# Vanlightly/vsr-tlaplus

Hardware: AMD Instinct MI355X
Metric: distinct states/sec (whole node) + time-to-first-violation, VSR 3-replica (higher is better)
Workload: dtype u64

## Files before the change

include/vsrmc.h:

```cpp
#ifndef VSRMC_H
#define VSRMC_H
#include <stdint.h>

#ifdef __cplusplus
extern "C" {
#endif

#define VSRMC_E_ARG (-1)
#define VSRMC_E_CFG (-2)
#define VSRMC_E_HIP (-3)
#define VSRMC_E_EVAL (-4)
#define VSRMC_E_REP (-5)
#define VSRMC_E_STATE (-6)

typedef struct vsrmc_model vsrmc_model;
typedef struct vsrmc_fpset vsrmc_fpset;
typedef struct vsrmc_checker vsrmc_checker;

const char* vsrmc_last_error(void);
int32_t vsrmc_version(void);
int32_t vsrmc_device_count(void);

typedef struct vsrmc_layout {
  int32_t replica_count, client_count, value_count, start_view_on_timer_limit;
// ... 217 lines not shown
  uint64_t min_fp[8], min_index[8];
  uint32_t min_ordinal[8];
  int32_t min_action[8];
  double kernel_ms, list_ms, apply_ms;
  uint64_t slices;
} vsrmc_step_info;
int32_t vsrmc_step_compile(const vsrmc_model* m, const char* text, vsrmc_where** out);
int32_t vsrmc_step_predicates_compile(const vsrmc_model* m, const char* text, vsrmc_where** out);
int32_t vsrmc_step_batch(const vsrmc_model* m, int32_t device, const vsrmc_where* w, const uint64_t* words, const uint64_t* off, uint64_t n, uint64_t* rows,
                         uint64_t cap_rows, uint64_t* n_rows);
int32_t vsrmc_checker_step_scan(vsrmc_checker* c, const vsrmc_where* w, vsrmc_step_info* out);
int32_t vsrmc_checker_step_successor(vsrmc_checker* c, uint64_t index, uint32_t ordinal, const uint64_t* parent, uint64_t parent_words, uint64_t* words,
                                     uint64_t cap_words, uint64_t* n_words, int32_t* action);
int32_t vsrmc_checker_step_pairs(vsrmc_checker* c, uint64_t* fps, uint32_t* ordinals, uint8_t* bits, uint64_t cap, uint64_t* n);

int32_t vsrmc_checker_probe(vsrmc_checker* c, vsrmc_level_info* info);
int32_t vsrmc_checker_probe2(vsrmc_checker* c, vsrmc_level_info* virt, vsrmc_level_info* probe);
int32_t vsrmc_checker_probe3(vsrmc_checker* c, vsrmc_level_info* virt1, vsrmc_level_info* virt2, vsrmc_level_info* probe);
int32_t vsrmc_checker_deepen(vsrmc_checker* c, vsrmc_level_info* inserted, vsrmc_level_info* probed);
int32_t vsrmc_checker_advance(vsrmc_checker* c, vsrmc_level_info* a, vsrmc_level_info* b, int32_t* what);
int32_t vsrmc_checker_room(vsrmc_checker* c, int32_t* state);
int32_t vsrmc_checker_probe_candidates(vsrmc_checker* c, uint64_t* pairs, uint64_t cap_pairs, uint64_t* n);
int32_t vsrmc_checker_probe_violators(vsrmc_checker* c, uint64_t* fps, uint64_t cap, uint64_t* n);
int32_t vsrmc_checker_seen_batch(vsrmc_checker* c, const uint64_t* fps, uint64_t n, int32_t level, uint8_t* seen);
int32_t vsrmc_checker_probe_trace(vsrmc_checker* c, uint64_t* words, uint64_t cap_words, uint64_t* off, int32_t* actions,
                                  uint64_t cap_states, uint64_t* n_states);
int32_t vsrmc_checker_trace_to_violator(vsrmc_checker* c, uint64_t fp, uint64_t* words, uint64_t cap_words, uint64_t* off, int32_t* actions,
                                        uint64_t cap_states, uint64_t* n_states);

typedef struct vsrmc_deep_info {
  int32_t level, kind;
  int32_t exact;
  int32_t has_state, has_step, reserved0;
  uint64_t slices;
  uint64_t n_hit_states, n_hit_pairs;
  double where_ms, step_ms;
} vsrmc_deep_info;
int32_t vsrmc_checker_deep_attach(vsrmc_checker* c, const vsrmc_where* state_prog, const vsrmc_where* step_prog);
int32_t vsrmc_checker_deep_levels(vsrmc_checker* c, int32_t* levels, int32_t* probed, uint64_t cap, uint64_t* n);
int32_t vsrmc_checker_deep_result(vsrmc_checker* c, int32_t level, int32_t probed, vsrmc_deep_info* info, vsrmc_where_info* w, vsrmc_step_info* s);
int32_t vsrmc_checker_deep_where_states(vsrmc_checker* c, int32_t level, int32_t probed, uint64_t* fps, uint8_t* bits, uint64_t cap, uint64_t* n);
int32_t vsrmc_checker_deep_step_pairs(vsrmc_checker* c, int32_t level, uint64_t* fps, uint32_t* ordinals, uint8_t* bits, uint64_t cap, uint64_t* n);
int32_t vsrmc_checker_deep_witness(vsrmc_checker* c, int32_t level, int32_t which_program, int32_t k, uint64_t* words, uint64_t cap_words, uint64_t* off,
                                   int32_t* actions, uint64_t cap_states, uint64_t* n_states);

typedef struct vsrmc_deep_terminal_info {
// ... 129 lines not shown
```

vsr_tlaplus_amd/capi.py:

```python
import ctypes as C
import os

HERE = os.path.dirname(os.path.abspath(__file__))
LIB_PATH = os.environ.get("VSRMC_LIB") or os.path.join(HERE, "libvsrmc.so")

u64p = C.POINTER(C.c_uint64)


class Layout(C.Structure):
    _fields_ = [(n, C.c_int32) for n in (
        "replica_count", "client_count", "value_count", "start_view_on_timer_limit", "symmetry", "invariant_mask",
        "assume_commit_number", "check_deadlock", "words_per_replica", "fixed_words", "permutations", "max_bag",
        "max_record_words", "module")] + [("reserved", C.c_int32 * 2)]


class Options(C.Structure):
    _fields_ = [("device", C.c_int32), ("table_log2", C.c_int32), ("frontier_words", C.c_uint64),
                ("frontier_states", C.c_uint64), ("pending_entries", C.c_uint64), ("keep_trace", C.c_int32),
                ("rank", C.c_int32), ("world", C.c_int32), ("trace_entries", C.c_uint64), ("exact_ties", C.c_int32), ("filter_log2", C.c_int32), ("host_frontier", C.c_int32), ("reserved0", C.c_int32), ("frontier_words_b", C.c_uint64)]


class LevelInfo(C.Structure):
    _fields_ = [("level", C.c_int32), ("error_code", C.c_int32), ("frontier", C.c_uint64), ("generated", C.c_uint64),
                ("n_new", C.c_uint64), ("distinct", C.c_uint64), ("total_generated", C.c_uint64),
# ... 189 lines not shown
    "vsrmc_checker_deep_terminal_states": (C.c_int32, [V, C.c_int32, C.c_int32, V, V, C.c_uint64, C.POINTER(C.c_uint64)]),
    "vsrmc_checker_deep_terminal_witness": (C.c_int32, [V, C.c_int32, C.c_int32, C.c_int32, V, C.c_uint64, V, V, C.c_uint64, C.POINTER(C.c_uint64)]),
    "vsrmc_check": (C.c_int32, [V, C.c_int32, C.c_double, C.POINTER(C.c_int32), C.POINTER(LevelInfo)]),
    "vsrmc_queue_create": (C.c_int32, [C.c_int32, C.c_uint64, C.c_uint64, C.POINTER(V)]),
    "vsrmc_queue_enqueue_batch": (C.c_int32, [V, V, V, C.c_uint64]),
    "vsrmc_queue_dequeue_batch": (C.c_int32, [V, C.c_uint64, V, C.c_uint64, V, C.POINTER(C.c_uint64)]),
    "vsrmc_queue_size": (C.c_int32, [V, C.POINTER(C.c_uint64)]),
    "vsrmc_queue_destroy": (None, [V]),
    "vsrmc_simulate": (C.c_int32, [V, C.c_int32, C.c_uint32, C.c_int32, C.c_uint64, C.c_double, C.POINTER(SimResult)]),
    "vsrmc_simulate_where": (C.c_int32, [V, C.c_int32, V, V, C.c_int32, C.c_uint32, C.c_int32, C.c_uint64, C.c_double, C.c_uint64,
                                         C.POINTER(SimWhereResult)]),
    "vsrmc_simulate_constrained": (C.c_int32, [V, C.c_int32, V, C.c_int32, V, C.c_int32, C.c_uint32, C.c_int32, C.c_uint32, C.c_int32, C.c_uint64,
                                               C.c_double, C.c_uint64, C.POINTER(SimConstrainedResult)]),
    "vsrmc_checker_probe": (C.c_int32, [V, C.POINTER(LevelInfo)]),
    "vsrmc_checker_probe2": (C.c_int32, [V, C.POINTER(LevelInfo), C.POINTER(LevelInfo)]),
    "vsrmc_checker_probe3": (C.c_int32, [V, C.POINTER(LevelInfo), C.POINTER(LevelInfo), C.POINTER(LevelInfo)]),
    "vsrmc_checker_deepen": (C.c_int32, [V, C.POINTER(LevelInfo), C.POINTER(LevelInfo)]),
    "vsrmc_checker_options": (C.c_int32, [V, C.POINTER(Options)]),
    "vsrmc_checker_advance": (C.c_int32, [V, C.POINTER(LevelInfo), C.POINTER(LevelInfo), C.POINTER(C.c_int32)]),
    "vsrmc_checker_room": (C.c_int32, [V, C.POINTER(C.c_int32)]),
    "vsrmc_checker_probe_candidates": (C.c_int32, [V, C.c_void_p, C.c_uint64, C.POINTER(C.c_uint64)]),
    "vsrmc_checker_seen_batch": (C.c_int32, [V, C.c_void_p, C.c_uint64, C.c_int32, C.c_void_p]),
    "vsrmc_checker_probe_violators": (C.c_int32, [V, C.c_void_p, C.c_uint64, C.POINTER(C.c_uint64)]),
    "vsrmc_checker_probe_trace": (C.c_int32, [V, V, C.c_uint64, V, V, C.c_uint64, C.POINTER(C.c_uint64)]),
    "vsrmc_checker_bench_staging": (C.c_int32, [V, C.c_int32, C.c_int32, C.POINTER(C.c_double), C.POINTER(C.c_uint64)]),
    "vsrmc_checker_trace_to_violator": (C.c_int32, [V, C.c_uint64, V, C.c_uint64, V, V, C.c_uint64, C.POINTER(C.c_uint64)]),
    "vsrmc_checker_save": (C.c_int32, [V, C.c_char_p]),
    "vsrmc_checker_status": (C.c_int32, [V, C.POINTER(LevelInfo)]),
    "vsrmc_checker_load": (C.c_int32, [V, C.POINTER(Options), C.c_char_p, C.POINTER(V)]),
    "vsrmc_model_parse_states": (C.c_int32, [V, C.c_char_p, V, C.c_uint64, V, V, C.c_uint64, C.POINTER(C.c_uint64)]),
    "vsrmc_model_check_trace": (C.c_int32, [V, C.c_int32, V, V, C.c_uint64, V, V, C.POINTER(C.c_int64), C.POINTER(C.c_int32)]),
    "vsrmc_shard_expand": (C.c_int32, [V, C.POINTER(ShardIO), V]),
    "vsrmc_shard_claim": (C.c_int32, [V, V, C.c_uint64, V]),
    "vsrmc_shard_materialize": (C.c_int32, [V, C.POINTER(ShardIO), V]),
    "vsrmc_shard_count": (C.c_int32, [V, C.POINTER(C.c_uint64), C.POINTER(C.c_uint64)]),
    "vsrmc_shard_export": (C.c_int32, [V, C.c_uint64, C.c_uint64, V, C.c_uint64, V, V, C.c_uint64, C.POINTER(C.c_uint64),
                                      C.POINTER(C.c_uint64)]),
    "vsrmc_shard_append": (C.c_int32, [V, V, C.c_uint64, V, V, C.c_uint64]),
    "vsrmc_shard_commit": (C.c_int32, [V, C.POINTER(LevelInfo)]),
    "vsrmc_shard_local_step": (C.c_int32, [V, C.POINTER(LevelInfo)]),
    "vsrmc_shard_partition": (C.c_int32, [V, C.POINTER(C.c_uint64)]),
    "vsrmc_shard_set_max_bag": (C.c_int32, [V, C.c_uint64]),
    "vsrmc_comm_rccl_unique_id": (C.c_int32, [V]),
    "vsrmc_comm_rccl_create": (C.c_int32, [V, C.c_int32, C.c_int32, C.c_int32, C.POINTER(C.POINTER(Comm))]),
    "vsrmc_comm_rccl_destroy": (None, [C.POINTER(Comm)]),
    "vsrmc_shard_loop_create": (C.c_int32, [V, C.POINTER(Comm), C.c_uint64, C.c_uint64, C.c_uint64, C.c_uint64, C.POINTER(V)]),
# ... 73 lines not shown
```

vsr_tlaplus_amd/checker.py:

```python
import ctypes as C
import os

import numpy as np

from . import capi
from .capi import VsrmcError, check

ACTION_NAMES = ["Initial predicate", "TimerSendSVC", "ReceiveHigherSVC", "ReceiveMatchingSVC", "SendDVC",
                "ReceiveHigherDVC", "ReceiveMatchingDVC", "SendSV", "ReceiveSV", "ReceiveClientRequest",
                "ReceivePrepareMsg", "ReceivePrepareOkMsg", "ExecuteOp", "SendGetState", "ReceiveGetState",
                "ReceiveNewState"]

INV_ACK_NOT_LOST = 1
INV_ACK_ON_MAJORITY = 2


def _p(a):
    return C.c_void_p(a.ctypes.data)


class Where:

    def __init__(self, handle, model):
        self._h = handle
# ... 1146 lines not shown
            self.violation = dict(level=d["level"], index=None, fp=d["viol_fp"], mask=d["viol_mask"], probed=True)
        return d

    def probe2(self):
        v, p = capi.LevelInfo(), capi.LevelInfo()
        check(capi.load().vsrmc_checker_probe2(self._h, C.byref(v), C.byref(p)))
        dv, dp = v.as_dict(), p.as_dict()
        for d in (dv, dp):
            d["ancestor_index"] = d.pop("viol_index")
            if d["viol_mask"] and self.violation is None:
                self.violation = dict(level=d["level"], index=None, fp=d["viol_fp"], mask=d["viol_mask"], probed=True)
        return dv, dp

    def probe3(self):
        v1, v2, p = capi.LevelInfo(), capi.LevelInfo(), capi.LevelInfo()
        check(capi.load().vsrmc_checker_probe3(self._h, C.byref(v1), C.byref(v2), C.byref(p)))
        out = [v1.as_dict(), v2.as_dict(), p.as_dict()]
        for d in out:
            d["ancestor_index"] = d.pop("viol_index")
            if d["viol_mask"] and self.violation is None:
                self.violation = dict(level=d["level"], index=None, fp=d["viol_fp"], mask=d["viol_mask"], probed=True)
        return tuple(out)

    def probe_violators(self):
        n = C.c_uint64()
        check(capi.load().vsrmc_checker_probe_violators(self._h, None, 0, C.byref(n)))
        out = np.zeros(max(1, n.value), dtype=np.uint64)
        check(capi.load().vsrmc_checker_probe_violators(self._h, _p(out), len(out), C.byref(n)))
        return [int(x) for x in out[: n.value]]

    def probe_trace(self):
        lay = self.model.layout
        n_max = max(self.level, self.depth) + 3
        cap_w = (n_max + 1) * int(lay.max_record_words)
        words = np.zeros(cap_w, dtype=np.uint64)
        off = np.zeros(n_max + 2, dtype=np.uint64)
        acts = np.zeros(n_max + 2, dtype=np.int32)
        n = C.c_uint64()
        check(capi.load().vsrmc_checker_probe_trace(self._h, _p(words), cap_w, _p(off), _p(acts), len(off), C.byref(n)))
        return [(ACTION_NAMES[acts[t]], words[int(off[t]): int(off[t + 1])].copy()) for t in range(n.value)]

    def trace_to_violator(self, fp):
        lay = self.model.layout
        n_max = max(self.level, self.depth) + 3
        cap_w = (n_max + 1) * int(lay.max_record_words)
        words = np.zeros(cap_w, dtype=np.uint64)
# ... 17 lines not shown
```

vsr_tlaplus_amd/csrc/host_checker.hpp:

```cpp
#pragma once

struct PassDst {
  u64* words = nullptr;
  u64 words_cap = 0;
  u64* off = nullptr;
  u64* fp = nullptr;
  u64 cap = 0;
  bool own_words = true;
  bool own_index = true;
};
struct DeepLevelRec { u64 n_new = 0, n_local = 0, generated = 0, max_bag = 0, frontier = 0; };
struct vsrmc_deep_attach;
struct vsrmc_deep_terminal;
struct vsrmc_constraint;
struct vsrmc_action_constraint;
struct vsrmc_checker {
  vsrmc_model model;
  vsrmc_options opt;
  hipStream_t stream = nullptr;
  hipEvent_t ev[4] = {nullptr, nullptr, nullptr, nullptr};
  Slot* table = nullptr;
  u64 tmask = 0;
  u64* words[2] = {nullptr, nullptr};
  u64* off[2] = {nullptr, nullptr};
// ... 12 lines not shown
  double t_level0 = 0, expand_ms = 0, materialize_ms = 0;
  u64 nx_n = 0, nx_w = 0;
  u64 n_valid = 1;
  u64 cur_w = 0;
  u64* rslot = nullptr;
  u64 rslot_cap = 0;
  u64* filter = nullptr;
  u64 fmask = 0;
  u64* cand_idx = nullptr;
  u64 cand_idx_cap = 0;
  bool level_fused = false;
  int failed_code = 0;
  void* fused_kernel = nullptr;
  void* plain_kernel = nullptr;
  u64* redo_buf[2] = {nullptr, nullptr};
  void* plain5_kernel = nullptr;
  void* modes_kernel = nullptr;
  void* regen_bits_kernel = nullptr, *insert_kernel = nullptr;
  void* probe_kernel = nullptr;
  void* probe_scan_kernel = nullptr, *probe_apply_kernel = nullptr;
  u64* probe_list = nullptr;
  u64 probe_list_cap = 0;
  bool probe_scan_off = false;
  u64 cur_max_bag = 0;
  bool bag_known = true;
  u64 probe_fp = 0, probe_extra_fp = 0;
  int probe_level = 0;
  std::vector<u64> probe_viol;
  std::vector<u64> probe_viol_key;
  int probe_viol_level = 0;
  int host_frontier = 0;
  bool saw_violation = false;
  u64 extra_launches = 0;
  bool probe_all_actions = false;
  int deep = 0;
  std::vector<DeepLevelRec> deep_lv;
  u64 deep_g = 2;
  u64 deep_distinct = 0, deep_generated = 0;
  bool deep_regen_done = false;
  bool rebase_off = false;
  std::vector<PassDst> scratch;
  PassDst scratch0;
  bool scratch_carved = false;
  int scratch_buf = -1;
  u64 scratch_front = 0;
  WSet h_wset = {nullptr, nullptr, 0};
// ... 50 lines not shown
double constraint_write_ratio(const vsrmc_checker* c);
bool deep_constrain_on(const vsrmc_checker* c);
int deep_constrain_filtered_through(const vsrmc_checker* c);
int deep_constrain_begin(vsrmc_checker* c, int first, int last);
int deep_constrain_slice(vsrmc_checker* c, const PassDst& B, u64 part, int level, ConstrainCtl* inserted);
int deep_constrain_end(vsrmc_checker* c, int rc, int base, int last_regen);
void deep_constrain_drop_empty(vsrmc_checker* c);
u64 deep_constrain_pruned_of(const vsrmc_checker* c, int level);
int phase_expand_gated(vsrmc_checker* c);
void action_constraint_restart(vsrmc_checker* c);
void action_constraint_free(vsrmc_checker* c);
int action_constraint_trace(vsrmc_checker* c, const std::vector<u64>& fps, u64* words, u64 cap_words, u64* off, int32_t* actions, u64 cap_states, u64* n_states);
const vsrmc_where* action_constraint_program(const vsrmc_checker* c, int* k);
bool action_deep_on(const vsrmc_checker* c);
int expand_pass_gated(vsrmc_checker* c, const u64* src_words, const u64* src_off, u64 n, u64 p_off, int level, int mode, u64 bag, const PassDst* dst);
void action_deep_file(vsrmc_checker* c, int level, int kind);
void action_deep_epoch(vsrmc_checker* c);
typedef void (*ExpandKernel)(Model, const u64*, const u64*, u64, int, int, Slot*, u64, u64*, u64, LevelCtl*, int, int, u64*, u64, u32, u64*,
                             u64, u64*, u64, u64*, u32, u32, int, u32, u64*, u64, u64*, u32, int, u64, const WSet*, u32);
typedef void (*MaterializeKernel)(Model, const u64*, const u64*, const u64*, u64, Slot*, u64*, u64, u64*, u64, u64*, LevelCtl*,
                                  const uint8_t*, u64*, u64*, int, u32, u32, int, const u64*);
typedef void (*ProbeScanKernel)(Model, const u64*, const u64*, u64, LevelCtl*, int, u32, u64*, u64);
typedef void (*ProbeApplyKernel)(Model, const u64*, const u64*, const u64*, u64, u64*, u64, LevelCtl*);
struct KernelSet {
  ExpandKernel exact;
  MaterializeKernel materialize;
  ExpandKernel fused;
  bool generic;
  ExpandKernel plain = nullptr, plain5 = nullptr, modes = nullptr, regen_bits = nullptr, insert = nullptr, probe = nullptr;
  ProbeScanKernel scan = nullptr;
  ProbeApplyKernel apply = nullptr;
};
template <int SPEC>
KernelSet full_set(ExpandKernel plain5 = nullptr) {
  KernelSet k{k_expand<false, SPEC>, k_materialize<SPEC>, k_expand<true, SPEC>, false, k_expand<true, SPEC, EXPAND_PLAIN>, plain5,
              k_expand<true, SPEC, EXPAND_MODES>, k_expand<true, SPEC, EXPAND_REGEN_BITS>, k_expand<true, SPEC, EXPAND_INSERT>};
  if constexpr ((SPEC % 1000) / 100 <= 3) { k.scan = k_probe_scan<SPEC>; k.apply = k_probe_apply<SPEC>; }
  else k.probe = k_expand<true, SPEC, EXPAND_PROBE>;
  return k;
}
KernelSet kernels_for(const Model& M) {
  switch (M.model_id * 1000 + M.R * 100 + M.C * 10 + M.n) {
    case 211: return {k_expand<false, 211>, k_materialize<211>, k_expand<true, 211>, false};
    case 212: return {k_expand<false, 0>, k_materialize<0>, k_expand<true, 212>, false};
    case 311: return {k_expand<false, 0>, k_materialize<0>, k_expand<true, 311>, false};
    case 312: return full_set<312>(k_expand<true, 312, EXPAND_PLAIN5>);
    case 313: return full_set<313>();
    case 323: {
      KernelSet k{k_expand<false, 0>, k_materialize<0>, k_expand<true, 323>, false};
      k.plain = k_expand<true, 323, EXPAND_PLAIN>;
      return k;
    }
    case 412: return {k_expand<false, 0>, k_materialize<0>, k_expand<true, 412>, false};
    case 512: return full_set<512>();
    case 1302: {
      KernelSet k{k_expand<false, 1000>, k_materialize<1000>, k_expand<true, 1302>, false};
      k.plain = k_expand<true, 1302, EXPAND_PLAIN>;
      return k;
    }
    case 2302: {
// ... 302 lines not shown
    vsrmc_checker_destroy(c);
    return fail(VSRMC_E_HIP, std::string("hipMalloc: ") + hipGetErrorString(e));
  }
  const KernelSet ks = kernels_for(M);
  c->fused_kernel = (void*)ks.fused;
  c->modes_kernel = (void*)ks.modes;
  c->plain_kernel = (void*)ks.plain;
  c->plain5_kernel = (void*)ks.plain5;
  c->regen_bits_kernel = (void*)ks.regen_bits;
  c->insert_kernel = (void*)ks.insert;
  c->probe_kernel = std::getenv("VSRMC_NO_PROBE_KERNEL") ? nullptr : (void*)ks.probe;
  if (ks.scan && ks.apply && !std::getenv("VSRMC_NO_PROBE_KERNEL")) {
    u64 cap = std::max<u64>((u64)1 << 12, std::min<u64>((u64)1 << 24, o->frontier_states / 4));
    if (const char* ev = std::getenv("VSRMC_PROBE_LIST")) cap = (u64)std::max<long long>(1, std::atoll(ev));
    if (hipMalloc((void**)&c->probe_list, ((u64)PSCAN_LIST_HDR + cap) * 8) == hipSuccess) {
      c->probe_list_cap = cap;
      c->probe_scan_kernel = (void*)ks.scan;
      c->probe_apply_kernel = (void*)ks.apply;
    } else {
      (void)hipGetLastError();
      c->probe_list = nullptr;
    }
  }
  rc = checker_seed(c);
  if (rc) { vsrmc_checker_destroy(c); return rc; }
  *out = c;
  return 0;
}

int32_t vsrmc_checker_options(const vsrmc_checker* c, vsrmc_options* out) {
  if (!c || !out) return fail(VSRMC_E_ARG, "NULL argument");
  *out = c->opt;
  return 0;
}

int32_t vsrmc_checker_reset(vsrmc_checker* c) {
  if (!c) return fail(VSRMC_E_ARG, "NULL argument");
  return checker_seed(c);
}

}

namespace {

int level_error(vsrmc_checker* c, const LevelCtl& h, int new_level) {
  c->failed = 1;
// ... 432 lines not shown
        return rrc;
      }
      return probe_pass_finish(c, src_words, src_off, level);
    }
    u32 cchunk = 0;
    if (io) {
      if (c->cand_idx_cap < (u64)c->opt.world * io->cand_cap) {
        if (c->cand_idx) (void)hipFree(c->cand_idx);
        c->cand_idx = nullptr;
        c->cand_idx_cap = 0;
        HIPCHK(hipMalloc((void**)&c->cand_idx, (u64)c->opt.world * io->cand_cap * 8));
        c->cand_idx_cap = (u64)c->opt.world * io->cand_cap;
      }
      cchunk = (u32)std::max<u64>(16, std::min<u64>(512, io->cand_cap / (4 * (u64)c->num_cus * 2)));
    }
    const int tile = fs.tile;
    const u64 ntiles = (n_parents + tile - 1) / tile;
    const u32 ccap = fs.ccap;
    const size_t lds = fs.lds;
    const int nxt = c->cur ^ 1;
    u64* const d_words = dst ? dst->words : c->words[nxt];
    u64* const d_off = dst ? dst->off : c->off[nxt];
    u64* const d_fp = dst ? dst->fp : c->lvl_fp;
    const u64 d_wcap = dst ? dst->words_cap : c->words_cap(nxt);
    const u64 nx_cap = dst ? dst->cap : c->opt.frontier_states;
    unsigned grid = (unsigned)std::min<u64>(ntiles, (u64)c->num_cus * fs.blocks_per_cu);
    grid = (unsigned)std::max<u64>(1, std::min<u64>(grid, std::min<u64>(nx_cap / (4 * (u64)VSR_CAND_CAP), d_wcap / (4 * 16384))));
    const u64 wmin = std::max<u64>(16384, (u64)ccap * (u64)(fs.stride + 5));
    grid = (unsigned)std::max<u64>(1, std::min<u64>(grid, d_wcap / (4 * wmin)));
    const u64 ichunk_max = (dst || mode == MODE_REGEN) ? std::max<u64>(VSR_CAND_CAP, 2048) : 8192;
    const u32 ichunk = (u32)std::max<u64>(VSR_CAND_CAP, std::min<u64>(ichunk_max, nx_cap / (4 * (u64)grid)));
    const u32 wchunk = (u32)std::max<u64>(std::min<u64>(wmin, d_wcap / 2), std::min<u64>(262144, d_wcap / (4 * (u64)grid)));
    HIPCHK(hipEventRecord(c->ev[0], c->stream));
    const void* kern = !one_rank ? c->fused_kernel : (use_plain || use_probe) ? fs.kernel : (c->modes_kernel ? c->modes_kernel : c->fused_kernel);
    if (!claim_bits && c->claim_bits && one_rank && level == c->level + 1 && (mode == MODE_INSERT || mode == MODE_REGEN) &&
        p_offset + n_parents <= c->claim_parents) { claim_bits = c->claim_bits; claim_w = c->claim_w; }
    if (one_rank && !use_plain) {
      if (mode == MODE_REGEN && claim_bits && c->regen_bits_kernel && claim_w <= 2 * (u64)(VSR_BLOCK / fs.tile)) kern = c->regen_bits_kernel;
      else if (mode == MODE_INSERT && c->insert_kernel) kern = c->insert_kernel;
    }
    if (claim_bits && kern != c->regen_bits_kernel && kern != c->insert_kernel) { claim_bits = nullptr; claim_w = 0; }
    if (use_plain || use_probe) { redo_kern = kern; redo_stride = fs.stride; redo_ichunk = ichunk; redo_wchunk = wchunk; redo_words = d_words; redo_off = d_off; redo_fp = d_fp; redo_wcap = d_wcap; redo_cap = nx_cap; redo_grid = grid; }
    hipLaunchKernelGGL((ExpandKernel)kern, dim3(grid), dim3(VSR_BLOCK), lds, c->stream, M, src_words, src_off, n_parents, level, c->opt.rank,
                       c->table, c->tmask, c->pending, c->opt.pending_entries, c->ctl, fs.stride, io ? c->opt.world : 1,
                       io ? io->cand_send : nullptr, io ? io->cand_cap : (u64)0, (u32)VSR_CAND_CAP,
                       d_words, d_wcap, d_off, nx_cap, d_fp,
                       ichunk, wchunk, tile, ccap, !one_rank ? c->filter : (u64*)claim_bits, !one_rank ? c->fmask : claim_w, io ? c->cand_idx : nullptr, cchunk,
                       mode | ((mode == MODE_PROBE && (c->saw_violation || c->probe_all_actions)) ? (int)MODE_NO_FOOTPRINT : 0), p_offset,
                       (const WSet*)((io && c->opt.world > 1) ? c->d_wset : nullptr), c->wepoch);
    HIPCHK(hipGetLastError());
    HIPCHK(hipEventRecord(c->ev[1], c->stream));
  }
  HIPCHK(hipMemcpyAsync(&c->h, c->ctl, sizeof(c->h), hipMemcpyDeviceToHost, c->stream));
  HIPCHK(hipStreamSynchronize(c->stream));
  if (n_parents > 0) {
    float ms = 0;
    HIPCHK(hipEventElapsedTime(&ms, c->ev[0], c->ev[1]));
    c->expand_ms += ms;
  }
  if (redo_kern && !use_probe && c->h.n_redo && !c->h.err) {
    const int rrc = redo_overflowed_tiles(c, redo_kern, src_words, src_off, level, redo_stride, redo_words, redo_wcap, redo_off, redo_cap, redo_fp, redo_ichunk, redo_wchunk, redo_grid);
    if (rrc) return rrc;
  }
  if (use_probe && c->h.n_redo > c->h.redo_cap && !c->h.err) c->h.err = ERR_FRONTIER_FULL;
  if (use_probe && c->h.n_redo && !c->h.err) {
    const int rrc = redo_overflowed_tiles(c, c->probe_kernel, src_words, src_off, level, redo_stride, redo_words, redo_wcap, redo_off, redo_cap, redo_fp, redo_ichunk, redo_wchunk,
                                          redo_grid, MODE_PROBE, probe_ccap);
    if (rrc) return rrc;
  }
  if (use_probe && c->h.err == ERR_FRONTIER_FULL) {
    void* const pk = c->probe_kernel;
    const u64 before = c->extra_launches + 1;
// ... 61 lines not shown
```

vsr_tlaplus_amd/csrc/host_search.hpp:

```cpp
#pragma once

extern "C" {

int32_t vsrmc_checker_probe(vsrmc_checker* c, vsrmc_level_info* info) {
  if (!c || !info) return fail(VSRMC_E_ARG, "NULL argument");
  if (c->opt.exact_ties) return fail(VSRMC_E_STATE, "probe levels need a single-pass checker");
  if (c->constraint && !deep_constrain_on(c)) return fail(VSRMC_E_STATE, "vsrmc_checker_probe: a constraint is attached (vsrmc_checker_constrain_attach): the levels beyond the record buffers are not constrained");
  if (c->action_constraint && !action_deep_on(c)) return fail(VSRMC_E_STATE, "vsrmc_checker_probe: an action constraint is attached (vsrmc_checker_action_constrain_attach): the levels beyond the record buffers are not constrained");
  if (c->action_constraint && c->constraint) return fail(VSRMC_E_STATE, "vsrmc_checker_probe: a state constraint beside an action constraint that is applied beyond the record buffers: the two together are not taken there");
  if (c->failed && c->failed_code != ERR_FRONTIER_FULL) return fail(VSRMC_E_STATE, "the checker stopped on an error");
  c->failed = 0;
  c->probe_fp = 0;
  c->probe_level = 0;
  c->probe_extra_fp = 0;
  c->probe_viol.clear();
  c->probe_viol_key.clear();
  c->probe_viol_level = 0;
  const bool gated = action_deep_on(c);
  int rc = 0;
  if (gated) {
    HIPCHK(hipSetDevice(c->opt.device));
    c->t_level0 = now_s();
    c->expand_ms = 0;
    action_deep_epoch(c);
// ... 60 lines not shown
  return 0;
}

int32_t vsrmc_checker_probe_candidates(vsrmc_checker* c, uint64_t* pairs, uint64_t cap_pairs, uint64_t* n) {
  if (!c || !n) return fail(VSRMC_E_ARG, "NULL argument");
  *n = c->h.n_pending;
  if (c->h.n_pending > c->opt.pending_entries) return fail(VSRMC_E_REP, "more violating successors than the pending list holds (pending_entries)");
  if (c->h.n_pending == 0 || !pairs) return 0;
  if (cap_pairs < c->h.n_pending) return fail(VSRMC_E_ARG, "buffer too small");
  HIPCHK(hipSetDevice(c->opt.device));
  HIPCHK(hipMemcpy(pairs, c->pending, 16 * c->h.n_pending, hipMemcpyDeviceToHost));
  return 0;
}

int32_t vsrmc_checker_probe_violators(vsrmc_checker* c, uint64_t* fps, uint64_t cap, uint64_t* n) {
  if (!c || !n) return fail(VSRMC_E_ARG, "NULL argument");
  *n = (u64)c->probe_viol.size();
  if (!fps) return 0;
  if (cap < *n) return fail(VSRMC_E_ARG, "buffer too small");
  for (u64 i = 0; i < *n; i++) fps[i] = c->probe_viol[(size_t)i];
  return 0;
}

int32_t vsrmc_checker_seen_batch(vsrmc_checker* c, const uint64_t* fps, uint64_t n, int32_t level, uint8_t* seen) {
  if (!c || (n && (!fps || !seen))) return fail(VSRMC_E_ARG, "NULL argument");
  if (n == 0) return 0;
  HIPCHK(hipSetDevice(c->opt.device));
  u64* d = nullptr;
  HIPCHK(hipMalloc((void**)&d, 16 * n));
  std::vector<u64> flags(n, 0);
  hipError_t e = hipMemcpy(d, fps, 8 * n, hipMemcpyHostToDevice);
  if (e == hipSuccess) {
    hipLaunchKernelGGL(k_table_seen, dim3((unsigned)((n + 255) / 256)), dim3(256), 0, c->stream, c->table, c->tmask, d, (u64)n, (int)level, d + n);
    e = hipGetLastError();
  }
  if (e == hipSuccess) e = hipStreamSynchronize(c->stream);
  if (e == hipSuccess) e = hipMemcpy(flags.data(), d + n, 8 * n, hipMemcpyDeviceToHost);
  (void)hipFree(d);
  if (e != hipSuccess) return fail(VSRMC_E_HIP, std::string("vsrmc_checker_seen_batch: ") + hipGetErrorString(e));
  for (u64 i = 0; i < n; i++) seen[i] = flags[i] ? 1 : 0;
  return 0;
}

int32_t vsrmc_checker_probe_trace(vsrmc_checker* c, uint64_t* words, uint64_t cap_words, uint64_t* off, int32_t* actions,
                                  uint64_t cap_states, uint64_t* n_states) {
  if (!c || !words || !off || !actions || !n_states) return fail(VSRMC_E_ARG, "NULL argument");
// ... 286 lines not shown
```

vsr_tlaplus_amd/csrc/vsrmc.hip:

```cpp
#include <algorithm>
#include <chrono>
#include <cstdio>
#include <cstdlib>
#include <cstring>
#include <fstream>
#include <map>
#include <sstream>
#include <string>
#include <vector>

#include "../../include/vsrmc.h"
#include "vsr_format.hpp"
#include "vrst_format.hpp"
#include "vras_format.hpp"
#include "vsr_parse.hpp"
#include "vras_parse.hpp"
#include "vsr_kernels.hpp"
#include "vsr_probe_scan.hpp"
#include "vsr_terminal.hpp"
#include "vsr_where.hpp"
#include "vsr_constrain.hpp"
#include "vsr_deep_constrain.hpp"
#include "vsr_where_parse.hpp"
#include "vsr_step.hpp"
#include "vsr_action_constrain.hpp"
#include "vsr_deep_where.hpp"
#include "vsr_deep_terminal.hpp"
#include "vsr_sim_where.hpp"
#include "vsr_sim_constrain.hpp"

#define VSRMC_FP_VERSION 2

using namespace vsr;

namespace {

thread_local std::string g_err;

int fail(int code, const std::string& msg) {
  g_err = msg;
  return code;
// ... 86 lines not shown
```

Measured before the change: 1.838 billion.

## Add dedicated wave-parallel regen-bits kernel driven by claim bitmaps

```diff
diff --git a/include/vsrmc.h b/include/vsrmc.h
--- a/include/vsrmc.h
+++ b/include/vsrmc.h
@@ -263,6 +263,7 @@
 int32_t vsrmc_checker_room(vsrmc_checker* c, int32_t* state);
 int32_t vsrmc_checker_probe_candidates(vsrmc_checker* c, uint64_t* pairs, uint64_t cap_pairs, uint64_t* n);
 int32_t vsrmc_checker_probe_violators(vsrmc_checker* c, uint64_t* fps, uint64_t cap, uint64_t* n);
+int32_t vsrmc_checker_regen_launches(const vsrmc_checker* c, uint64_t* n);
 int32_t vsrmc_checker_seen_batch(vsrmc_checker* c, const uint64_t* fps, uint64_t n, int32_t level, uint8_t* seen);
 int32_t vsrmc_checker_probe_trace(vsrmc_checker* c, uint64_t* words, uint64_t cap_words, uint64_t* off, int32_t* actions,
                                   uint64_t cap_states, uint64_t* n_states);
diff --git a/vsr_tlaplus_amd/capi.py b/vsr_tlaplus_amd/capi.py
--- a/vsr_tlaplus_amd/capi.py
+++ b/vsr_tlaplus_amd/capi.py
@@ -235,6 +235,7 @@
     "vsrmc_checker_probe_candidates": (C.c_int32, [V, C.c_void_p, C.c_uint64, C.POINTER(C.c_uint64)]),
     "vsrmc_checker_seen_batch": (C.c_int32, [V, C.c_void_p, C.c_uint64, C.c_int32, C.c_void_p]),
     "vsrmc_checker_probe_violators": (C.c_int32, [V, C.c_void_p, C.c_uint64, C.POINTER(C.c_uint64)]),
+    "vsrmc_checker_regen_launches": (C.c_int32, [V, C.POINTER(C.c_uint64)]),
     "vsrmc_checker_probe_trace": (C.c_int32, [V, V, C.c_uint64, V, V, C.c_uint64, C.POINTER(C.c_uint64)]),
     "vsrmc_checker_bench_staging": (C.c_int32, [V, C.c_int32, C.c_int32, C.POINTER(C.c_double), C.POINTER(C.c_uint64)]),
     "vsrmc_checker_trace_to_violator": (C.c_int32, [V, C.c_uint64, V, C.c_uint64, V, V, C.c_uint64, C.POINTER(C.c_uint64)]),
diff --git a/vsr_tlaplus_amd/checker.py b/vsr_tlaplus_amd/checker.py
--- a/vsr_tlaplus_amd/checker.py
+++ b/vsr_tlaplus_amd/checker.py
@@ -1192,6 +1192,11 @@
                 self.violation = dict(level=d["level"], index=None, fp=d["viol_fp"], mask=d["viol_mask"], probed=True)
         return tuple(out)
 
+    def regen_launches(self):
+        n = C.c_uint64()
+        check(capi.load().vsrmc_checker_regen_launches(self._h, C.byref(n)))
+        return n.value
+
     def probe_violators(self):
         n = C.c_uint64()
         check(capi.load().vsrmc_checker_probe_violators(self._h, None, 0, C.byref(n)))
diff --git a/vsr_tlaplus_amd/csrc/host_checker.hpp b/vsr_tlaplus_amd/csrc/host_checker.hpp
--- a/vsr_tlaplus_amd/csrc/host_checker.hpp
+++ b/vsr_tlaplus_amd/csrc/host_checker.hpp
@@ -58,6 +58,10 @@
   u64* probe_list = nullptr;
   u64 probe_list_cap = 0;
   bool probe_scan_off = false;
+  void* regen_kernel = nullptr;
+  u32 regen_trip = 64;
+  u64 regen_launches = 0;
+  u64 regen_dst_states = 0, regen_dst_words = 0;
   u64 cur_max_bag = 0;
   bool bag_known = true;
   u64 probe_fp = 0, probe_extra_fp = 0;
@@ -154,6 +158,7 @@
                                   const uint8_t*, u64*, u64*, int, u32, u32, int, const u64*);
 typedef void (*ProbeScanKernel)(Model, const u64*, const u64*, u64, LevelCtl*, int, u32, u64*, u64);
 typedef void (*ProbeApplyKernel)(Model, const u64*, const u64*, const u64*, u64, u64*, u64, LevelCtl*);
+typedef void (*RegenBitsKernel)(Model, const u64*, const u64*, u64, u64, const u32*, u32, LevelCtl*, int, u32, u32, u64*, u64, u64*, u64, u64*, u32, u32);
 struct KernelSet {
   ExpandKernel exact;
   MaterializeKernel materialize;
@@ -162,12 +167,13 @@
   ExpandKernel plain = nullptr, plain5 = nullptr, modes = nullptr, regen_bits = nullptr, insert = nullptr, probe = nullptr;
   ProbeScanKernel scan = nullptr;
   ProbeApplyKernel apply = nullptr;
+  RegenBitsKernel regen = nullptr;
 };
 template <int SPEC>
 KernelSet full_set(ExpandKernel plain5 = nullptr) {
   KernelSet k{k_expand<false, SPEC>, k_materialize<SPEC>, k_expand<true, SPEC>, false, k_expand<true, SPEC, EXPAND_PLAIN>, plain5,
               k_expand<true, SPEC, EXPAND_MODES>, k_expand<true, SPEC, EXPAND_REGEN_BITS>, k_expand<true, SPEC, EXPAND_INSERT>};
-  if constexpr ((SPEC % 1000) / 100 <= 3) { k.scan = k_probe_scan<SPEC>; k.apply = k_probe_apply<SPEC>; }
+  if constexpr ((SPEC % 1000) / 100 <= 3) { k.scan = k_probe_scan<SPEC>; k.apply = k_probe_apply<SPEC>; k.regen = k_regen_bits<SPEC>; }
   else k.probe = k_expand<true, SPEC, EXPAND_PROBE>;
   return k;
 }
@@ -516,6 +522,10 @@
       c->probe_list = nullptr;
     }
   }
+  if (ks.regen && !std::getenv("VSRMC_NO_REGEN_KERNEL")) c->regen_kernel = (void*)ks.regen;
+  if (const char* ev = std::getenv("VSRMC_REGEN_TRIP")) c->regen_trip = (u32)std::max(1, std::min(64, std::atoi(ev)));
+  if (const char* ev = std::getenv("VSRMC_REGEN_DST_STATES")) c->regen_dst_states = (u64)std::max<long long>(2 * VSR_CAND_CAP, std::atoll(ev));
+  if (const char* ev = std::getenv("VSRMC_REGEN_DST_WORDS")) c->regen_dst_words = (u64)std::max<long long>(1 << 17, std::atoll(ev));
   rc = checker_seed(c);
   if (rc) { vsrmc_checker_destroy(c); return rc; }
   *out = c;
@@ -994,8 +1004,9 @@
     u64* const d_words = dst ? dst->words : c->words[nxt];
     u64* const d_off = dst ? dst->off : c->off[nxt];
     u64* const d_fp = dst ? dst->fp : c->lvl_fp;
-    const u64 d_wcap = dst ? dst->words_cap : c->words_cap(nxt);
-    const u64 nx_cap = dst ? dst->cap : c->opt.frontier_states;
+    const bool cut_dst = mode == MODE_REGEN && !io;
+    const u64 d_wcap = std::min<u64>(dst ? dst->words_cap : c->words_cap(nxt), cut_dst && c->regen_dst_words ? c->regen_dst_words : ~(u64)0);
+    const u64 nx_cap = std::min<u64>(dst ? dst->cap : c->opt.frontier_states, cut_dst && c->regen_dst_states ? c->regen_dst_states : ~(u64)0);
     unsigned grid = (unsigned)std::min<u64>(ntiles, (u64)c->num_cus * fs.blocks_per_cu);
     grid = (unsigned)std::max<u64>(1, std::min<u64>(grid, std::min<u64>(nx_cap / (4 * (u64)VSR_CAND_CAP), d_wcap / (4 * 16384))));
     const u64 wmin = std::max<u64>(16384, (u64)ccap * (u64)(fs.stride + 5));
@@ -1012,7 +1023,26 @@
       else if (mode == MODE_INSERT && c->insert_kernel) kern = c->insert_kernel;
     }
     if (claim_bits && kern != c->regen_bits_kernel && kern != c->insert_kernel) { claim_bits = nullptr; claim_w = 0; }
+    if (kern == c->regen_bits_kernel && claim_bits && c->regen_kernel && fs.tile == 64 && claim_w <= (u64)RGB_ROW_WORDS && c->lds_stride <= 65) {
+      const size_t dyn = rgb_lds_bytes(fs.stride);
+      int nb = 0;
+      if (hipOccupancyMaxActiveBlocksPerMultiprocessor(&nb, c->regen_kernel, VSR_BLOCK, dyn) != hipSuccess || nb < 1) return fail(VSRMC_E_HIP, "k_regen_bits: no resident block");
+      const u64 nmt = (n_parents + RGB_MT - 1) / RGB_MT;
+      const u64 wmin_w = (u64)64 * (u64)c->lds_stride;
+      u64 rgrid = std::max<u64>(1, std::min<u64>((nmt + 3) / 4, (u64)c->num_cus * (u64)std::min(nb, (int)VSR_OCC)));
+      rgrid = std::max<u64>(1, std::min<u64>(rgrid, std::min<u64>(nx_cap / (16 * 64), d_wcap / (16 * wmin_w))));
+      const u32 r_ichunk = (u32)std::max<u64>(64, std::min<u64>(RGB_ICHUNK, nx_cap / (16 * rgrid)));
+      const u32 r_wchunk = (u32)std::max<u64>(wmin_w, std::min<u64>(RGB_WCHUNK, d_wcap / (16 * rgrid)));
+      if (16 * (u64)r_ichunk <= nx_cap && 16 * (u64)r_wchunk <= d_wcap) {
+        const u32 draw = nmt >= rgrid * 4 * RGB_DRAW * 4 ? (u32)RGB_DRAW : 1u;
+        hipLaunchKernelGGL((RegenBitsKernel)c->regen_kernel, dim3((unsigned)rgrid), dim3(VSR_BLOCK), dyn, c->stream, M, src_words, src_off, n_parents, p_offset,
+                           (const u32*)claim_bits, (u32)claim_w, c->ctl, fs.stride, draw, c->regen_trip, d_words, d_wcap, d_off, nx_cap, d_fp, r_ichunk, r_wchunk);
+        c->regen_launches++;
+        kern = nullptr;
+      }
+    }
     if (use_plain || use_probe) { redo_kern = kern; redo_stride = fs.stride; redo_ichunk = ichunk; redo_wchunk = wchunk; redo_words = d_words; redo_off = d_off; redo_fp = d_fp; redo_wcap = d_wcap; redo_cap = nx_cap; redo_grid = grid; }
+    if (kern) {
     hipLaunchKernelGGL((ExpandKernel)kern, dim3(grid), dim3(VSR_BLOCK), lds, c->stream, M, src_words, src_off, n_parents, level, c->opt.rank,
                        c->table, c->tmask, c->pending, c->opt.pending_entries, c->ctl, fs.stride, io ? c->opt.world : 1,
                        io ? io->cand_send : nullptr, io ? io->cand_cap : (u64)0, (u32)VSR_CAND_CAP,
@@ -1020,6 +1050,7 @@
                        ichunk, wchunk, tile, ccap, !one_rank ? c->filter : (u64*)claim_bits, !one_rank ? c->fmask : claim_w, io ? c->cand_idx : nullptr, cchunk,
                        mode | ((mode == MODE_PROBE && (c->saw_violation || c->probe_all_actions)) ? (int)MODE_NO_FOOTPRINT : 0), p_offset,
                        (const WSet*)((io && c->opt.world > 1) ? c->d_wset : nullptr), c->wepoch);
+    }
     HIPCHK(hipGetLastError());
     HIPCHK(hipEventRecord(c->ev[1], c->stream));
   }
diff --git a/vsr_tlaplus_amd/csrc/host_search.hpp b/vsr_tlaplus_amd/csrc/host_search.hpp
--- a/vsr_tlaplus_amd/csrc/host_search.hpp
+++ b/vsr_tlaplus_amd/csrc/host_search.hpp
@@ -106,6 +106,12 @@
   return 0;
 }
 
+int32_t vsrmc_checker_regen_launches(const vsrmc_checker* c, uint64_t* n) {
+  if (!c || !n) return fail(VSRMC_E_ARG, "NULL argument");
+  *n = c->regen_launches;
+  return 0;
+}
+
 int32_t vsrmc_checker_seen_batch(vsrmc_checker* c, const uint64_t* fps, uint64_t n, int32_t level, uint8_t* seen) {
   if (!c || (n && (!fps || !seen))) return fail(VSRMC_E_ARG, "NULL argument");
   if (n == 0) return 0;
diff --git a/vsr_tlaplus_amd/csrc/regen_ord.hpp b/vsr_tlaplus_amd/csrc/regen_ord.hpp
--- /dev/null
+++ b/vsr_tlaplus_amd/csrc/regen_ord.hpp
@@ -0,0 +1,33 @@
+#pragma once
+
+#ifndef REGEN_ORD_FN
+#define REGEN_ORD_FN inline
+#endif
+
+enum { REGEN_ORD_TIMER_SEND_SVC = 0, REGEN_ORD_SEND_DVC = 1, REGEN_ORD_SEND_SV = 2, REGEN_ORD_EXECUTE_OP = 3, REGEN_ORD_CLIENT_REQUEST = 4, REGEN_ORD_MESSAGE = 5 };
+
+struct RegenOrd {
+  int cls;
+  int r;
+  int b;
+  int j, k2;
+};
+
+REGEN_ORD_FN int regen_ord_m0(int R, int C, int n) { return 4 * R + R * C * n; }
+
+REGEN_ORD_FN RegenOrd regen_ord(int R, int C, int n, int ord) {
+  RegenOrd o = {REGEN_ORD_MESSAGE, 0, 0, 0, 0};
+  const int m0 = regen_ord_m0(R, C, n);
+  if (ord < 4 * R) {
+    o.cls = ord / R;
+    o.r = ord % R + 1;
+  } else if (ord < m0) {
+    o.cls = REGEN_ORD_CLIENT_REQUEST;
+    o.r = (ord - 4 * R) / (C * n) + 1;
+    o.b = (ord - 4 * R) % (C * n);
+  } else {
+    o.j = (ord - m0) / (R + 1);
+    o.k2 = (ord - m0) % (R + 1);
+  }
+  return o;
+}
diff --git a/vsr_tlaplus_amd/csrc/vsr_regen_bits.hpp b/vsr_tlaplus_amd/csrc/vsr_regen_bits.hpp
--- /dev/null
+++ b/vsr_tlaplus_amd/csrc/vsr_regen_bits.hpp
@@ -0,0 +1,298 @@
+#pragma once
+#include "vsr_kernels.hpp"
+#define REGEN_ORD_FN __host__ __device__ __forceinline__
+#include "regen_ord.hpp"
+
+
+namespace vsr {
+
+constexpr int RGB_MT = 16;
+constexpr int RGB_DRAW = 16;
+constexpr int RGB_ROW_WORDS = 8;
+constexpr int RGB_WAVE_EXTRA = RGB_MT + 64 / 2 + 2 * 64 / 2;
+constexpr u32 RGB_ICHUNK = 512;
+constexpr u32 RGB_WCHUNK = 32768;
+__host__ __device__ __forceinline__ size_t rgb_lds_bytes(int stride) { return (size_t)(VSR_BLOCK / 64) * (size_t)(RGB_MT * stride + RGB_WAVE_EXTRA) * 8; }
+
+template <int SPEC>
+__global__ void __launch_bounds__(VSR_BLOCK, VSR_OCC)
+k_regen_bits(Model Marg, const u64* __restrict__ fr_words, const u64* __restrict__ fr_off, u64 n_parents, u64 p_offset ,
+             const u32* __restrict__ claim_bits, u32 claim_w, LevelCtl* ctl, int stride, u32 draw ,
+             u32 trip , u64* nx_words, u64 nx_words_cap, u64* nx_off, u64 nx_cap, u64* lvl_fp,
+             u32 ichunk , u32 wchunk ) {
+  static_assert(SPEC / 1000 == 0 && SPEC % 1000 != 0 && (SPEC % 1000) / 100 <= 3, "VSR.tla, R <= 3: a record fits 64 words");
+  typedef ModelOps<0> Ops;
+  Model M = Marg;
+  specialise<SPEC>(M, Marg);
+  extern __shared__ u64 smem[];
+  __shared__ unsigned long long s_sum[3];
+  const int lane = threadIdx.x & 63, wave = threadIdx.x >> 6;
+  u64* const s_rec = smem + wave * (RGB_MT * stride + RGB_WAVE_EXTRA);
+  u64* const s_ref = s_rec + RGB_MT * stride;
+  u32* const s_pre = (u32*)(s_ref + RGB_MT);
+  u32* const s_bits = s_pre + 64;
+  if (threadIdx.x < 3) s_sum[threadIdx.x] = 0;
+  __syncthreads();
+
+  const u64 nmt = (n_parents + RGB_MT - 1) / RGB_MT;
+  const u64 lt_mask = ((u64)1 << lane) - 1;
+  u64 n_written = 0, rec_words = 0;
+  u32 maxbag = 0;
+  u64 idx_base = 0, w_base = 0;
+  u32 idx_left = 0, w_left = 0;
+
+  u64 cur = 0, nxt_v = 0;
+  u32 left = 0;
+  if (lane == 0) nxt_v = atomicAdd((unsigned long long*)&ctl->tile_cursor, 1ull);
+  auto next_mt = [&]() -> u64 {
+    if (left == 0) {
+      cur = readlane64(nxt_v, 0) * (u64)draw;
+      left = draw;
+      if (lane == 0 && cur < nmt) nxt_v = atomicAdd((unsigned long long*)&ctl->tile_cursor, 1ull);
+    }
+    left--;
+    return cur++;
+  };
+  const int l16 = lane & 15, q0 = lane >> 4;
+  auto load_ref = [&](u64 mt) -> u64 {
+    const u64 idx = mt * RGB_MT + (u64)l16;
+    return (mt < nmt && idx < n_parents) ? fr_off[idx] : 0;
+  };
+  auto spread = [&](u64 ref1, u64* refq) {
+#pragma unroll
+    for (int q = 0; q < 4; q++) {
+      const u32 lo = (u32)__shfl((int)(u32)ref1, q0 + 4 * q), hi = (u32)__shfl((int)(u32)(ref1 >> 32), q0 + 4 * q);
+      refq[q] = ((u64)hi << 32) | lo;
+    }
+  };
+  auto load_words = [&](u64 ref1, u64 (*v)[4]) {
+    u64 refq[4];
+    spread(ref1, refq);
+#pragma unroll
+    for (int q = 0; q < 4; q++) {
+      const u64 off = refq[q] >> 8;
+      const int len = (int)(refq[q] & 255) < stride ? (int)(refq[q] & 255) : stride;
+#pragma unroll
+      for (int j = 0; j < 4; j++) {
+        const int k = l16 + 16 * j;
+        v[q][j] = k < len ? fr_words[off + k] : 0;
+      }
+    }
+  };
+  const int bp = lane >> 2, bw = lane & 3;
+  auto load_bits = [&](u64 mt, u32* cb) {
+    const u64 idx = mt * RGB_MT + (u64)bp;
+    cb[0] = cb[1] = 0;
+    if (mt < nmt && idx < n_parents) {
+      const u32* row = claim_bits + (p_offset + idx) * (u64)claim_w;
+      if ((u32)bw < claim_w) cb[0] = row[bw];
+      if ((u32)bw + 4 < claim_w) cb[1] = row[bw + 4];
+    }
+  };
+
+  u64 refA, refB, v[4][4];
+  u32 cbA[2], cbB[2];
+  u64 mt0 = next_mt();
+  refA = load_ref(mt0);
+  load_bits(mt0, cbA);
+  u64 mt1 = next_mt();
+  refB = load_ref(mt1);
+  while (mt0 < nmt) {
+    load_words(refA, v);
+    {
+      u64 refq[4];
+      spread(refA, refq);
+#pragma unroll
+      for (int q = 0; q < 4; q++) {
+        const int p = q0 + 4 * q;
+        const int len = (int)(refq[q] & 255) < stride ? (int)(refq[q] & 255) : stride;
+#pragma unroll
+        for (int j = 0; j < 4; j++) {
+          const int k = l16 + 16 * j;
+          if (k < len) s_rec[p * stride + k] = v[q][j];
+        }
+      }
+      if (lane < RGB_MT) s_ref[lane] = refA;
+    }
+    const u32 cb0 = cbA[0], cb1 = cbA[1];
+    load_bits(mt1, cbB);
+    refA = refB;
+    cbA[0] = cbB[0];
+    cbA[1] = cbB[1];
+    const u64 mt2 = next_mt();
+    refB = load_ref(mt2);
+    lds_wave_sync();
+
+    const u64 p_base = mt0 * RGB_MT;
+    u32 total;
+    {
+      const u64 ref = s_ref[bp];
+      const bool fits = (int)(ref & 255) <= stride;
+      const bool valid = p_base + (u64)bp < n_parents && ref != 0 && fits;
+      if (!fits && bw == 0) raise_error(ctl, ERR_INTERNAL, (p_base + (u64)bp) << 16);
+      const u32 b0 = valid ? cb0 : 0u, b1 = valid ? cb1 : 0u;
+      u32 incl = (u32)__popc(b0) + (u32)__popc(b1);
+#pragma unroll
+      for (int o = 1; o < 64; o <<= 1) {
+        const u32 t = __shfl_up(incl, o);
+        if (lane >= o) incl += t;
+      }
+      s_pre[lane] = incl;
+      s_bits[2 * lane] = b0;
+      s_bits[2 * lane + 1] = b1;
+      total = (u32)__builtin_amdgcn_readlane((int)incl, 63);
+    }
+    lds_wave_sync();
+
+    for (u32 first = 0; first < total; first += trip) {
+      const bool active = (u32)lane < trip && first + (u32)lane < total;
+      const u32 i = active ? first + (u32)lane : 0u;
+      int L = 0;
+#pragma unroll
+      for (int s = 32; s > 0; s >>= 1)
+        if (s_pre[L + s - 1] <= i) L += s;
+      u32 k = i - (L ? s_pre[L - 1] : 0u);
+      u64 w = (u64)s_bits[2 * L] | ((u64)s_bits[2 * L + 1] << 32);
+      if (!active) { w = 1; k = 0; }
+      for (; k; k--) w &= w - 1;
+      const int b = __ffsll((long long)w) - 1;
+      const int p = L >> 2;
+      const int ord = 32 * ((L & 3) + (b >= 32 ? 4 : 0)) + (b & 31);
+      const u64* rec = s_rec + p * stride;
+
+      bool ok = active;
+      Delta D;
+      u64 Hc[6];
+      u64 fp = 0;
+      int plen = 0, clen = 0;
+      if (active) {
+        const RegenOrd o = regen_ord(M.R, M.C, M.n, ord);
+        int kind;
+        if (o.cls != REGEN_ORD_MESSAGE) {
+          kind = o.cls == REGEN_ORD_TIMER_SEND_SVC ? A_TimerSendSVC : o.cls == REGEN_ORD_SEND_DVC ? A_SendDVC : o.cls == REGEN_ORD_SEND_SV ? A_SendSV
+               : o.cls == REGEN_ORD_EXECUTE_OP ? A_ExecuteOp : A_ReceiveClientRequest;
+        } else {
+          int kind0 = 0;
+          (void)Ops::guard(M, rec, M.m0 + o.j, &kind0);
+          kind = o.k2 == 0 ? kind0 : Ops::other_kind(kind0);
+        }
+        if (!Ops::template gen_<false>(M, rec, ord, D) || D.action != kind) {
+          raise_error(ctl, ERR_INTERNAL, ((p_base + (u64)p) << 16) | (u64)ord);
+          ok = false;
+        } else if (D.err) {
+          raise_error(ctl, D.err, ((p_base + (u64)p) << 16) | (u64)ord);
+          ok = false;
+        }
+      }
+      if (ok) {
+        Ops::hash_child_(M, rec, D, Hc);
+        u32 ak;
+        canonical_fp(M, D.hdr, Hc, &fp, &ak);
+        plen = (int)(s_ref[p] & 255);
+        clen = M.fixed + hdr_nmsg(D.hdr);
+        if ((u32)hdr_nmsg(D.hdr) > maxbag) maxbag = (u32)hdr_nmsg(D.hdr);
+      }
+
+      const u64 okm = __ballot(ok);
+      const u32 nwin = (u32)__popcll(okm);
+      if (nwin == 0) continue;
+      u32 wincl = (u32)clen;
+#pragma unroll
+      for (int o = 1; o < 64; o <<= 1) {
+        const u32 t = __shfl_up(wincl, o);
+        if (lane >= o) wincl += t;
+      }
+      const u32 wtotal = (u32)__builtin_amdgcn_readlane((int)wincl, 63);
+      if (idx_left < nwin) {
+        for (u32 t = (u32)lane; t < idx_left; t += 64) { nx_off[idx_base + t] = 0; lvl_fp[idx_base + t] = 0; }
+        u64 nb = 0;
+        if (lane == 0) {
+          nb = atomicAdd((unsigned long long*)&ctl->n_new, (unsigned long long)ichunk);
+          if (nb + ichunk > nx_cap) { raise_full(ctl, nb); nb = 0; }
+        }
+        idx_base = readlane64(nb, 0);
+        idx_left = ichunk;
+      }
+      const u64 idx = idx_base + (u64)__popcll(okm & lt_mask);
+      idx_base += nwin;
+      idx_left -= nwin;
+      const u64 fitm = __ballot(wincl <= w_left);
+      const u32 cut = fitm ? (u32)__builtin_amdgcn_readlane((int)wincl, 63 - __clzll((long long)fitm)) : 0u;
+      u64 dst = w_base + (u64)(wincl - (u32)clen);
+      if (cut < wtotal) {
+        u64 nb = 0;
+        if (lane == 0) {
+          nb = atomicAdd((unsigned long long*)&ctl->words_new, (unsigned long long)wchunk);
+          if (nb + wchunk > nx_words_cap) { raise_full(ctl, nb); nb = 0; }
+        }
+        nb = readlane64(nb, 0);
+        if (wincl > cut) dst = nb + (u64)(wincl - (u32)clen - cut);
+        w_base = nb + (u64)(wtotal - cut);
+        w_left = wchunk - (wtotal - cut);
+      } else {
+        w_base += wtotal;
+        w_left -= wtotal;
+      }
+      n_written += nwin;
+      rec_words += wtotal;
+
+      for (u64 wm = okm; wm;) {
+        const int l0 = __ffsll((long long)wm) - 1;
+        wm &= wm - 1;
+        const int l1 = wm ? __ffsll((long long)wm) - 1 : l0;
+        wm &= wm - 1;
+        const int n0 = __builtin_amdgcn_readlane(plen, l0), n1 = l1 != l0 ? __builtin_amdgcn_readlane(plen, l1) : 0;
+        const u64* r0 = s_rec + __builtin_amdgcn_readlane(p, l0) * stride;
+        const u64* r1 = s_rec + __builtin_amdgcn_readlane(p, l1) * stride;
+        u64* o0 = nx_words + readlane64(dst, l0);
+        u64* o1 = nx_words + readlane64(dst, l1);
+        for (int t = lane; t < n0 || t < n1; t += 64) {
+          const u64 v0 = t < n0 ? r0[t] : 0, v1 = t < n1 ? r1[t] : 0;
+          if (t < n0) o0[t] = v0;
+          if (t < n1) o1[t] = v1;
+        }
+      }
+      if (ok) {
+        u64* out = nx_words + dst;
+        out[0] = D.hdr;
+        u64* ob = out + 1 + (D.r - 1) * M.wpr;
+        ob[0] = D.rep[0];
+        if (M.wpr > 1) ob[1] = D.rep[1];
+        if (M.wpr > 2) ob[2] = D.rep[2];
+        if (M.wpr > 3) ob[3] = D.rep[3];
+#pragma unroll
+        for (int h = 0; h < 6; h++)
+          if (h < M.np) out[M.h0 + h] = Hc[h];
+        int a = 0;
+#pragma unroll
+        for (int s = 0; s < VSR_NSLOT; s++)
+          if ((D.used >> s) & 1) {
+            if (D.pj(s) >= 0) out[M.fixed + D.pj(s)] = D.pnew[s];
+            else out[plen + (a++)] = D.pnew[s];
+          }
+        nx_off[idx] = (dst << 8) | (u64)clen;
+        lvl_fp[idx] = fp;
+      }
+    }
+    lds_wave_sync();
+    mt0 = mt1;
+    mt1 = mt2;
+  }
+  for (u32 t = (u32)lane; t < idx_left; t += 64) { nx_off[idx_base + t] = 0; lvl_fp[idx_base + t] = 0; }
+#pragma unroll
+  for (int o = 32; o > 0; o >>= 1) {
+    const u32 t = __shfl_down(maxbag, o);
+    maxbag = t > maxbag ? t : maxbag;
+  }
+  if (lane == 0) {
+    if (n_written) atomicAdd(&s_sum[0], (unsigned long long)n_written);
+    if (rec_words) atomicAdd(&s_sum[1], (unsigned long long)rec_words);
+    if (maxbag) atomicMax(&s_sum[2], (unsigned long long)maxbag);
+  }
+  __syncthreads();
+  if (threadIdx.x == 0 && s_sum[0]) atomicAdd((unsigned long long*)&ctl->n_written, s_sum[0]);
+  if (threadIdx.x == 1 && s_sum[1]) atomicAdd((unsigned long long*)&ctl->rec_words, s_sum[1]);
+  if (threadIdx.x == 2 && s_sum[2]) atomicMax((unsigned long long*)&ctl->max_bag, s_sum[2]);
+}
+
+}
diff --git a/vsr_tlaplus_amd/csrc/vsrmc.hip b/vsr_tlaplus_amd/csrc/vsrmc.hip
--- a/vsr_tlaplus_amd/csrc/vsrmc.hip
+++ b/vsr_tlaplus_amd/csrc/vsrmc.hip
@@ -17,6 +17,7 @@
 #include "vras_parse.hpp"
 #include "vsr_kernels.hpp"
 #include "vsr_probe_scan.hpp"
+#include "vsr_regen_bits.hpp"
 #include "vsr_terminal.hpp"
 #include "vsr_where.hpp"
 #include "vsr_constrain.hpp"
```

Result: faster. 1.879 billion (median of 6 runs) (+2.3%).
